# Ankur-Deka/Emergent-Multiagent-Strategies

Measured on AMD Instinct MI355X. Metric: env-steps/sec FortAttack 3v3, 4096 parallel envs per GPU, higher is better.
Workload: dtype f64

## Files before the change

emergent-multiagent-strategies_amd/build.py:

```python
import os
import shutil
import subprocess

CSRC = os.path.join(os.path.dirname(os.path.abspath(__file__)), "csrc")
ROOT = os.path.dirname(os.path.dirname(os.path.abspath(__file__)))
LIB = os.path.join(CSRC, "libfortattack_hip.so")
if os.environ.get("FA_LIBRARY"):
    LIB = os.path.abspath(os.environ["FA_LIBRARY"])
OBJ = os.path.join(CSRC, "_obj")
SOURCES = ["fa_step_pipe.hip", "fa_step_classic.hip", "fa_collect.hip", "fa_policy.hip", "fa_attend.hip", "fa_train.hip", "fa_train_dw.hip", "fa_fold.hip", "fa_rccl.hip", "fa_api.hip"]
FLAGS = ["--offload-arch=gfx950", "-O3", "-std=c++17", "-ffp-contract=off", "-fPIC", "-shared"]


def hipcc():
    return shutil.which("hipcc") or "/opt/rocm/bin/hipcc"


def needs_build():
    if os.environ.get("FA_LIBRARY"):
        return False
    if not os.path.isfile(LIB):
        return True
    deps = [os.path.join(CSRC, f) for f in SOURCES + ["fa_device.h", "fa_step_common.h", "experiments/fa_step_experiments.h", "fa_probe.h", "fa_policy.h", "fa_mfma.h", "fa_train.h"]]
    deps.append(os.path.join(ROOT, "include", "fortattack.h"))
    return any(os.path.getmtime(d) > os.path.getmtime(LIB) for d in deps)


def _load_mod(fname):
    import importlib.util
    spec = importlib.util.spec_from_file_location("_fa_" + fname[:-3], os.path.join(os.path.dirname(os.path.abspath(__file__)), fname))
    mod = importlib.util.module_from_spec(spec)
    spec.loader.exec_module(mod)
    return mod


def _load_lint():
    return _load_mod("isa_lint.py")


def _compile_one(src, verbose):
    isa_lint = _load_lint()
    base = os.path.join(OBJ, os.path.splitext(src)[0])
    common = [hipcc()] + [f for f in FLAGS if f != "-shared"] + ["-I", os.path.join(ROOT, "include")]
    cmd = common + ["-c", os.path.join(CSRC, src), "-o", base + ".o"]
    if verbose:
        print(" ".join(cmd))
    subprocess.check_call(cmd)
    subprocess.check_call(common + ["-S", "--cuda-device-only", os.path.join(CSRC, src), "-o", base + ".s"])
    bad = isa_lint.lint(base + ".s")
    if bad:
        raise RuntimeError("isa_lint: %s has %d vector instruction(s) ahead of an exec restore (a misplaced live-range "
                           "split: lanes that skipped the region lose the value), first: %s %s line %d: %s"
                           % (src, len(bad), bad[0][0], bad[0][1], bad[0][2][0], bad[0][2][1]))
    return base + ".o"


def build(force=False, verbose=False):
    if os.environ.get("FA_LIBRARY") or (not force and not needs_build()):
        return LIB
    from concurrent.futures import ThreadPoolExecutor
    os.makedirs(OBJ, exist_ok=True)
    with ThreadPoolExecutor(max_workers=4) as pool:
        objs = list(pool.map(lambda f: _compile_one(f, verbose), SOURCES))
    isa_model = _load_mod("isa_model.py")
    m = isa_model.write(os.path.join(OBJ, "fa_step_pipe.s"), os.path.join(OBJ, "fa_isa_model.json"))
    if os.environ.get("FA_ISA_REFRESH") == "1":
        isa_model.write(os.path.join(OBJ, "fa_step_pipe.s"))
    bad = isa_model.check(m)
    if bad:
        msg = "isa_model: the shipped step-kernel instantiations regressed: " + "; ".join(bad)
        if os.environ.get("FA_ISA_GATE", "1") == "0":
            import warnings
            warnings.warn(msg + "  (FA_ISA_GATE=0: building anyway)")
        else:
            if os.path.isfile(LIB):
                os.remove(LIB)
            raise RuntimeError(msg + "  (FA_ISA_GATE=0 builds anyway)")
    cmd = [hipcc(), "--offload-arch=gfx950", "-fPIC", "-shared"] + objs + ["-o", LIB]
    if verbose:
        print(" ".join(cmd))
    subprocess.check_call(cmd)
    return LIB


if __name__ == "__main__":
    print(build(force=True, verbose=True))
```

emergent-multiagent-strategies_amd/csrc/fa_mfma.h:

```cpp
#pragma once
#include <hip/hip_runtime.h>
#include <stdint.h>

#include "fa_policy.h"

#ifndef FA_GEMM_CH
#define FA_GEMM_CH 8
#endif
namespace {
constexpr int LDA = 132;
typedef float f32x16 __attribute__((ext_vector_type(16)));

template <int K>
struct BHead {
    static constexpr int NT = K / 8;
    static constexpr int CH = NT < FA_GEMM_CH ? NT : FA_GEMM_CH;
    float4 v[CH];
};
template <int K>
__device__ __forceinline__ void prefetch_b(const float4 *__restrict__ wp, int lane, BHead<K> &h) {
#pragma unroll
    for (int c = 0; c < BHead<K>::CH; ++c) h.v[c] = wp[c * 64 + lane];
}

template <int K, int NRB>
__device__ __forceinline__ void gemm_cb(const float *arow, const float4 *__restrict__ wp, f32x16 (&acc)[NRB], int lane,
                                        const BHead<K> &head) {
    constexpr int NT = BHead<K>::NT, CH = BHead<K>::CH;
    float4 bq[CH], bn[CH];
#pragma unroll
    for (int c = 0; c < CH; ++c) bq[c] = head.v[c];
#pragma unroll
    for (int t0 = 0; t0 < NT; t0 += CH) {
        if (t0 + CH < NT) {
#pragma unroll
            for (int c = 0; c < CH; ++c) bn[c] = wp[(t0 + CH + c) * 64 + lane];
#ifndef FA_NO_SCHED_BARRIER
            __builtin_amdgcn_sched_barrier(0);
#endif
        }
#pragma unroll
        for (int c = 0; c < CH; ++c) {
#pragma unroll
            for (int r = 0; r < NRB; ++r) {
                const float4 a = *reinterpret_cast<const float4 *>(arow + r * 32 * LDA + (t0 + c) * 4);
                acc[r] = __builtin_amdgcn_mfma_f32_32x32x2f32(a.x, bq[c].x, acc[r], 0, 0, 0);
                acc[r] = __builtin_amdgcn_mfma_f32_32x32x2f32(a.y, bq[c].y, acc[r], 0, 0, 0);
                acc[r] = __builtin_amdgcn_mfma_f32_32x32x2f32(a.z, bq[c].z, acc[r], 0, 0, 0);
                acc[r] = __builtin_amdgcn_mfma_f32_32x32x2f32(a.w, bq[c].w, acc[r], 0, 0, 0);
            }
        }
        if (t0 + CH < NT) {
#pragma unroll
            for (int c = 0; c < CH; ++c) bq[c] = bn[c];
        }
    }
}

#ifndef FA_GEMM3_CH
#define FA_GEMM3_CH 1
#endif
typedef __bf16 fa_bf16x8 __attribute__((ext_vector_type(8)));
typedef unsigned fa_u32x4 __attribute__((ext_vector_type(4)));
template <int K>
struct BHead3 {
    static constexpr int NS = K / 16;
    static constexpr int CH = NS < FA_GEMM3_CH ? NS : FA_GEMM3_CH;
    fa_u32x4 v[CH * 3];
};
template <int K>
__device__ __forceinline__ void prefetch_b3(const fa_u32x4 *__restrict__ wp, int lane, BHead3<K> &h) {
#pragma unroll
    for (int c = 0; c < BHead3<K>::CH * 3; ++c) h.v[c] = wp[c * 64 + lane];
}
__device__ __forceinline__ void fa_split8(const float4 &a0, const float4 &a1, fa_u32x4 &H, fa_u32x4 &M, fa_u32x4 &L) {
    const float x[8] = {a0.x, a0.y, a0.z, a0.w, a1.x, a1.y, a1.z, a1.w};
    unsigned h[8], m[8], l[8];
#pragma unroll
    for (int j = 0; j < 8; ++j) {
        h[j] = __float_as_uint(x[j]) & 0xffff0000u;
        const float r1 = x[j] - __uint_as_float(h[j]);
        m[j] = __float_as_uint(r1) & 0xffff0000u;
        l[j] = __float_as_uint(r1 - __uint_as_float(m[j]));
    }
#pragma unroll
    for (int j = 0; j < 4; ++j) {
        H[j] = __builtin_amdgcn_perm(h[2 * j + 1], h[2 * j], 0x07060302u);
        M[j] = __builtin_amdgcn_perm(m[2 * j + 1], m[2 * j], 0x07060302u);
        L[j] = __builtin_amdgcn_perm(l[2 * j + 1], l[2 * j], 0x07060302u);
    }
}
template <int K, int NRB>
__device__ __forceinline__ void gemm_cb3(const float *arow, const fa_u32x4 *__restrict__ wp3, f32x16 (&acc)[NRB], int lane,
                                         const BHead3<K> &head) {
    constexpr int NS = BHead3<K>::NS, CH = BHead3<K>::CH;
    fa_u32x4 bq[CH * 3], bn[CH * 3];
#pragma unroll
    for (int c = 0; c < CH * 3; ++c) bq[c] = head.v[c];
#pragma unroll
    for (int s0 = 0; s0 < NS; s0 += CH) {
        if (s0 + CH < NS) {
#pragma unroll
#ifdef FA_X3_KO_WLOAD
            for (int c = 0; c < CH * 3; ++c) bn[c] = bq[c] ^ (unsigned)s0;
#else
            for (int c = 0; c < CH * 3; ++c) bn[c] = wp3[((s0 + CH) * 3 + c) * 64 + lane];
#endif
#ifndef FA_NO_SCHED_BARRIER
            __builtin_amdgcn_sched_barrier(0);
#endif
        }
#pragma unroll
        for (int c = 0; c < CH; ++c) {
            const fa_bf16x8 bh = __builtin_bit_cast(fa_bf16x8, bq[c * 3]), bm = __builtin_bit_cast(fa_bf16x8, bq[c * 3 + 1]),
                            bl = __builtin_bit_cast(fa_bf16x8, bq[c * 3 + 2]);
#pragma unroll
            for (int r = 0; r < NRB; ++r) {
                const float *ap = arow + r * 32 * LDA + (s0 + c) * 8;
                fa_u32x4 H, M, L;
#ifdef FA_X3_KO_SPLIT
                H = __builtin_bit_cast(fa_u32x4, *reinterpret_cast<const float4 *>(ap));
                M = __builtin_bit_cast(fa_u32x4, *reinterpret_cast<const float4 *>(ap + 4));
                L = H ^ M;
#else
                fa_split8(*reinterpret_cast<const float4 *>(ap), *reinterpret_cast<const float4 *>(ap + 4), H, M, L);
#endif
                const fa_bf16x8 ah = __builtin_bit_cast(fa_bf16x8, H), am = __builtin_bit_cast(fa_bf16x8, M),
                                al = __builtin_bit_cast(fa_bf16x8, L);
                acc[r] = __builtin_amdgcn_mfma_f32_32x32x16_bf16(ah, bl, acc[r], 0, 0, 0);
                acc[r] = __builtin_amdgcn_mfma_f32_32x32x16_bf16(al, bh, acc[r], 0, 0, 0);
                acc[r] = __builtin_amdgcn_mfma_f32_32x32x16_bf16(am, bm, acc[r], 0, 0, 0);
                acc[r] = __builtin_amdgcn_mfma_f32_32x32x16_bf16(ah, bm, acc[r], 0, 0, 0);
                acc[r] = __builtin_amdgcn_mfma_f32_32x32x16_bf16(am, bh, acc[r], 0, 0, 0);
                acc[r] = __builtin_amdgcn_mfma_f32_32x32x16_bf16(ah, bh, acc[r], 0, 0, 0);
            }
#if !defined(FA_NO_SCHED_BARRIER) && !defined(FA_X3_NO_STEP_FENCE)
            __builtin_amdgcn_sched_barrier(0);
#endif
        }
        if (s0 + CH < NS) {
#pragma unroll
            for (int c = 0; c < CH * 3; ++c) bq[c] = bn[c];
        }
    }
}

template <bool RELU>
__device__ __forceinline__ void store_acc(float *dst, int rb, const f32x16 &acc, float bias, int lane) {
    const int col = lane & 31, hh = lane >> 5;
#pragma unroll
    for (int reg = 0; reg < 16; ++reg) {
        const int row = rb * 32 + (reg & 3) + 8 * (reg >> 2) + 4 * hh;
        float v = acc[reg] + bias;
        if (RELU) v = fmaxf(v, 0.0f);
        dst[row * LDA + col] = v;
    }
}

__device__ __forceinline__ float group16_sum(float v) {
#define FA_ROR_ADD(n) v += __builtin_bit_cast(float, __builtin_amdgcn_update_dpp(0, __builtin_bit_cast(int, v), 0x120 | (n), 0xf, 0xf, false))
    FA_ROR_ADD(8);
    FA_ROR_ADD(4);
    FA_ROR_ADD(2);
    FA_ROR_ADD(1);
#undef FA_ROR_ADD
    return v;
}

template <int W>
__device__ __forceinline__ void attend_row(const float *grow, const float *key0, int nk, int skip, float *orow, int q,
                                           float *attn_row = nullptr) {
    constexpr int C = W / 16;
    float gv[C];
#pragma unroll
    for (int c = 0; c < C; c += 4) *reinterpret_cast<float4 *>(gv + c) = *reinterpret_cast<const float4 *>(grow + q * C + c);
    float s[FA_POLICY_MAX_TEAM];
    float mx = -INFINITY;
#pragma unroll
    for (int j = 0; j < FA_POLICY_MAX_TEAM; ++j) {
        s[j] = -INFINITY;
        if (j < nk && j != skip) {
            float kv[C];
#pragma unroll
            for (int c = 0; c < C; c += 4)
                *reinterpret_cast<float4 *>(kv + c) = *reinterpret_cast<const float4 *>(key0 + j * LDA + q * C + c);
            float d = 0.0f;
#pragma unroll
            for (int c = 0; c < C; ++c) d = fmaf(gv[c], kv[c], d);
            s[j] = group16_sum(d);
            mx = fmaxf(mx, s[j]);
        }
    }
    float den = 0.0f;
#pragma unroll
    for (int j = 0; j < FA_POLICY_MAX_TEAM; ++j) {
        s[j] = (j < nk && j != skip) ? __expf(s[j] - mx) : 0.0f;
        den += s[j];
    }
    const float inv = den > 0.0f ? 1.0f / den : 0.0f;
    float ov[C];
#pragma unroll
    for (int c = 0; c < C; ++c) ov[c] = 0.0f;
#pragma unroll
    for (int j = 0; j < FA_POLICY_MAX_TEAM; ++j) {
        if (j < nk && j != skip) {
            const float a = s[j] * inv;
#pragma unroll
            for (int c = 0; c < C; c += 4) {
                const float4 kv = *reinterpret_cast<const float4 *>(key0 + j * LDA + q * C + c);
                ov[c] = fmaf(a, kv.x, ov[c]);
                ov[c + 1] = fmaf(a, kv.y, ov[c + 1]);
                ov[c + 2] = fmaf(a, kv.z, ov[c + 2]);
                ov[c + 3] = fmaf(a, kv.w, ov[c + 3]);
            }
        }
    }
#pragma unroll
    for (int c = 0; c < C; c += 4) *reinterpret_cast<float4 *>(orow + q * C + c) = *reinterpret_cast<const float4 *>(ov + c);
    if (attn_row && q < nk) {
        float aq = s[0];
#pragma unroll
        for (int j = 1; j < FA_POLICY_MAX_TEAM; ++j) aq = (j == q) ? s[j] : aq;
        attn_row[q] = aq * inv;
    }
}

template <int W, int MT>
__device__ __forceinline__ void attend_row_regs(const float *grow, const float *key0, int nk, int skip, int q, float (&ov)[W / 16],
                                                float *attn_row = nullptr) {
    constexpr int C = W / 16;
    float gv[C], kv[MT][C];
#pragma unroll
    for (int c = 0; c < C; c += 4) *reinterpret_cast<float4 *>(gv + c) = *reinterpret_cast<const float4 *>(grow + q * C + c);
#pragma unroll
    for (int j = 0; j < MT; ++j) {
#pragma unroll
        for (int c = 0; c < C; c += 4)
            *reinterpret_cast<float4 *>(&kv[j][c]) = j < nk ? *reinterpret_cast<const float4 *>(key0 + j * LDA + q * C + c) : float4{0, 0, 0, 0};
    }
    float s[MT], mx = -INFINITY;
#pragma unroll
    for (int j = 0; j < MT; ++j) {
        float d = 0.0f;
#pragma unroll
        for (int c = 0; c < C; ++c) d = fmaf(gv[c], kv[j][c], d);
        s[j] = group16_sum(d);
    }
#pragma unroll
    for (int j = 0; j < MT; ++j) {
        s[j] = (j < nk && j != skip) ? s[j] : -INFINITY;
        mx = fmaxf(mx, s[j]);
    }
    float den = 0.0f;
#pragma unroll
    for (int j = 0; j < MT; ++j) {
        s[j] = (j < nk && j != skip) ? __expf(s[j] - mx) : 0.0f;
        den += s[j];
    }
    const float inv = den > 0.0f ? 1.0f / den : 0.0f;
#pragma unroll
    for (int c = 0; c < C; ++c) ov[c] = 0.0f;
#pragma unroll
    for (int j = 0; j < MT; ++j) {
        if (j < nk) {
            const float a = s[j] * inv;
#pragma unroll
            for (int c = 0; c < C; ++c) ov[c] = fmaf(a, kv[j][c], ov[c]);
        }
    }
    if (attn_row && q < nk) {
        float aq = s[0];
#pragma unroll
        for (int j = 1; j < MT; ++j) aq = (j == q) ? s[j] : aq;
        attn_row[q] = aq * inv;
    }
}
template <int W>
__device__ __forceinline__ void store_row_regs(float *orow, int q, const float (&ov)[W / 16]) {
    constexpr int C = W / 16;
#pragma unroll
    for (int c = 0; c < C; c += 4) *reinterpret_cast<float4 *>(orow + q * C + c) = *reinterpret_cast<const float4 *>(ov + c);
}

}
```

emergent-multiagent-strategies_amd/csrc/fa_policy.hip:

```cpp
#include <hip/hip_runtime.h>
#include <stdint.h>
#include <type_traits>

#include "fa_policy.h"
#include "fa_mfma.h"
#define FA_PROBE_POLICY_TU
#include "fa_probe.h"

#ifndef FA_POLICY_WAVES
#define FA_POLICY_WAVES 8
#endif
#ifndef FA_POLICY_X3
#define FA_POLICY_X3 1
#endif
namespace {
#if FA_POLICY_X3
typedef fa_u32x4 pw_t;
template <int K> using PBHead = BHead3<K>;
template <int K> __device__ __forceinline__ void p_prefetch(const pw_t *__restrict__ wp, int lane, PBHead<K> &h) { prefetch_b3<K>(wp, lane, h); }
template <int K, int NRB>
__device__ __forceinline__ void p_gemm(const float *arow, const pw_t *__restrict__ wp, f32x16 (&acc)[NRB], int lane, const PBHead<K> &h) {
    gemm_cb3<K, NRB>(arow, wp, acc, lane, h);
}
#define FA_PW(OFF, OFF3, K, cb) (reinterpret_cast<const pw_t *>(W + (OFF3)) + (size_t)(cb) * ((K) / 16) * 3 * 64)
#else
typedef float4 pw_t;
template <int K> using PBHead = BHead<K>;
template <int K> __device__ __forceinline__ void p_prefetch(const pw_t *__restrict__ wp, int lane, PBHead<K> &h) { prefetch_b<K>(wp, lane, h); }
template <int K, int NRB>
__device__ __forceinline__ void p_gemm(const float *arow, const pw_t *__restrict__ wp, f32x16 (&acc)[NRB], int lane, const PBHead<K> &h) {
    gemm_cb<K, NRB>(arow, wp, acc, lane, h);
}
#define FA_PW(OFF, OFF3, K, cb) (reinterpret_cast<const pw_t *>(W + (OFF)) + (size_t)(cb) * ((K) / 8) * 64)
#endif
__device__ __forceinline__ void philox4x32_10(uint32_t c[4], uint32_t k0, uint32_t k1) {
#pragma unroll
    for (int r = 0; r < 10; ++r) {
        uint32_t hi0 = __umulhi(0xD2511F53u, c[0]), lo0 = 0xD2511F53u * c[0];
        uint32_t hi1 = __umulhi(0xCD9E8D57u, c[2]), lo1 = 0xCD9E8D57u * c[2];
        uint32_t n0 = hi1 ^ c[1] ^ k0, n2 = hi0 ^ c[3] ^ k1;
        c[0] = n0; c[1] = lo1; c[2] = n2; c[3] = lo0;
        k0 += 0x9E3779B9u; k1 += 0xBB67AE85u;
    }
}

#define FA_WAVES_BARRIER() asm volatile("s_waitcnt lgkmcnt(0)\n\ts_barrier" ::: "memory")
#define FA_POLICY_SPLIT(...)                                                          \
    if constexpr (NW == 8) {                                                          \
        if (wave < 4) { constexpr int R0 = 0, NR = 2; __VA_ARGS__ }                   \
        else { constexpr int R0 = 2, NR = 1; __VA_ARGS__ }                            \
    } else if constexpr (NW == 12) {                                                  \
        const int R0 = wave >> 2; constexpr int NR = 1; __VA_ARGS__                   \
    } else { constexpr int R0 = 0, NR = NRB; __VA_ARGS__ }
template <int NRB, int NW, bool ATTN>
__global__ __launch_bounds__(NW * 64, NRB == 2 ? 2 : 1) void fa_policy_kernel(FaPolicyArgs a) {
    static_assert((NRB == 3 && (NW == 8 || NW == 12)) || NW == 4, "eight / twelve waves: the 96-row tile");
    constexpr int PR = 32 * NRB;
    constexpr int NT = NW * 64;
    __shared__ __attribute__((aligned(16))) float sH[PR * LDA];
    __shared__ __attribute__((aligned(16))) float sG[PR * LDA];
    __shared__ float sX[PR * 2 * FA_OBS_DIM];
    __shared__ float sO[PR * 16];
    __shared__ float sNz[NW == 8 ? PR * FA_NUM_ACTIONS : 1];

    const int tid = threadIdx.x, lane = tid & 63, wave = __builtin_amdgcn_readfirstlane(tid >> 6);
    const int team = blockIdx.y;
    const int N = a.G + a.A;
    const int n = team == 0 ? a.G : a.A, m = N - n;
    const int own0 = team == 0 ? 0 : a.G, opp0 = team == 0 ? a.G : 0;
    const int ET = PR / (n > m ? n : m);
    const unsigned inv_n = 65536u / (unsigned)n + 1u, inv_m = 65536u / (unsigned)m + 1u;
    auto div_n = [&](int r) { return (int)(((unsigned)r * inv_n) >> 16); };
    auto div_m = [&](int r) { return (int)(((unsigned)r * inv_m) >> 16); };
    __shared__ int sE[PR];
    const float *W = a.w[team];
    if (a.env_list) {
        const int strat = a.tile_strategy[blockIdx.x];
        if (strat < 0) return;
        if (team == 1) W = a.pool + (size_t)strat * FA_POLICY_WEIGHT_FLOATS;
        if (tid < ET) sE[tid] = a.env_list[blockIdx.x * ET + tid];
    } else {
        const int e0 = blockIdx.x * ET;
        if (e0 >= a.E) return;
        if (tid < ET) sE[tid] = e0 + tid < a.E ? e0 + tid : -1;
    }
    float we[FA_OBS_DIM], wo[FA_OBS_DIM];
#pragma unroll
    for (int k = 0; k < FA_OBS_DIM; ++k) {
        we[k] = W[FA_POFF_WE + k * 64 + (tid & 63)];
        wo[k] = W[FA_POFF_WOE + k * 64 + (tid & 63)];
    }
    const float be = W[FA_POFF_BE + (tid & 63)], bo = W[FA_POFF_BOE + (tid & 63)];
    __syncthreads();

    for (int k = tid; k < ET * N * FA_OBS_DIM; k += NT) {
        const int el = k / (N * FA_OBS_DIM), e = sE[el];
        sX[k] = e >= 0 ? a.obs[(size_t)e * N * FA_OBS_DIM + (k - el * N * FA_OBS_DIM)] : 0.0f;
    }
    __syncthreads();

    FA_PL_TICK(0)
    const int li = lane & 31, hh = lane >> 5;
    const int cbw = wave & 3;
    const bool opp_two = NW == 4 && NRB == 3 && wave < 2;
    const bool opp_on = NW == 4 || wave < 2 * NRB;
    const int ocb = wave & 1, orb = NW >= 8 ? (wave >> 1) : (NRB == 3 ? 2 : (wave >> 1));
    const pw_t *wp_ao = FA_PW(FA_POFF_AO, FA_POFF3_AO, 64, ocb);
    const pw_t *wp_bo = FA_PW(FA_POFF_BO, FA_POFF3_BO, 64, ocb);
    const pw_t *wp_am = FA_PW(FA_POFF_AM, FA_POFF3_AM, 128, cbw);
    const pw_t *wp_w7 = FA_PW(FA_POFF_W7, FA_POFF3_W7, 256, cbw);
    const pw_t *wp_w8p = FA_PW(FA_POFF_W8, FA_POFF3_W8, 128, cbw);
    const pw_t *wp_w8v = FA_PW(FA_POFF_W8, FA_POFF3_W8, 128, 4 + cbw);
    const pw_t *wp_w9 = FA_PW(FA_POFF_W9, FA_POFF3_W9, 256, 0);
    PBHead<64> hd_o;
    if (opp_on) p_prefetch<64>(wp_ao, lane, hd_o);
    {
        const int col = tid & 63, grp = tid >> 6;
        for (int r = grp; r < PR; r += NW) {
            float vo = 0.0f, vp = 0.0f;
            if (r < ET * n) {
                const int el = div_n(r), i = r - el * n;
                const float *x = sX + (el * N + own0 + i) * FA_OBS_DIM;
                vo = be;
#pragma unroll
                for (int k = 0; k < FA_OBS_DIM; ++k) vo = fmaf(x[k], we[k], vo);
                vo = fmaxf(vo, 0.0f);
            }
            if (r < ET * m) {
                const int el = div_m(r), j = r - el * m;
                const float *x = sX + (el * N + opp0 + j) * FA_OBS_DIM;
                vp = bo;
#pragma unroll
                for (int k = 0; k < FA_OBS_DIM; ++k) vp = fmaf(x[k], wo[k], vp);
                vp = fmaxf(vp, 0.0f);
            }
            sH[r * LDA + col] = vo;
            sG[r * LDA + col] = vp;
        }
    }
    __syncthreads();
    FA_PL_TICK(1)

    if (opp_two) {
        f32x16 acc[2] = {};
        p_gemm<64, 2>(sH + li * LDA + hh * 32, wp_ao, acc, lane, hd_o);
        p_prefetch<64>(wp_bo, lane, hd_o);
        store_acc<false>(sG + 64 + ocb * 32, 0, acc[0], 0.0f, lane);
        store_acc<false>(sG + 64 + ocb * 32, 1, acc[1], 0.0f, lane);
    } else if (opp_on) {
        f32x16 acc[1] = {};
        p_gemm<64, 1>(sH + (orb * 32 + li) * LDA + hh * 32, wp_ao, acc, lane, hd_o);
        p_prefetch<64>(wp_bo, lane, hd_o);
        store_acc<false>(sG + 64 + ocb * 32, orb, acc[0], 0.0f, lane);
    }
    __syncthreads();
    FA_PL_TICK(2)
    constexpr int AIT = PR / (NW * 4);
    const int q16 = lane & 15, arow0 = wave * 4 + (lane >> 4), RU = ET * n;
    const bool small_teams = (n > m ? n : m) <= 4, mid_teams = (n > m ? n : m) <= 6;
    auto attn_dst = [&](float *base, int r, int nk) -> float * {
        if (!base || r >= RU) return nullptr;
        const int el = div_n(r), e = sE[el];
        return e >= 0 ? base + ((size_t)e * n + (r - el * n)) * nk : nullptr;
    };
    auto opp_attention = [&](auto MTc) __attribute__((always_inline)) {
        constexpr int MT = decltype(MTc)::value;
        float ov[AIT][4];
#pragma unroll
        for (int k = 0; k < AIT; ++k) {
            const int r = arow0 + k * NW * 4, rr = r < RU ? r : RU - 1;
            if constexpr (ATTN)
                attend_row_regs<64, MT>(sG + rr * LDA + 64, sG + (div_n(rr) * m) * LDA, m, -1, q16, ov[k], attn_dst(a.opp_attn[team], r, m));
            else
                attend_row_regs<64, MT>(sG + rr * LDA + 64, sG + (div_n(rr) * m) * LDA, m, -1, q16, ov[k]);
        }
#pragma unroll
        for (int k = 0; k < AIT; ++k) {
            const int r = arow0 + k * NW * 4;
            if (r < RU) store_row_regs<64>(sG + r * LDA + 64, q16, ov[k]);
        }
    };
    if (small_teams) opp_attention(std::integral_constant<int, 4>{});
    else if (mid_teams) opp_attention(std::integral_constant<int, 6>{});
    else opp_attention(std::integral_constant<int, FA_POLICY_MAX_TEAM>{});
    __syncthreads();
    FA_PL_TICK(3)
    PBHead<128> hd_m;
    if (opp_two) {
        f32x16 acc[2] = {};
        p_gemm<64, 2>(sG + li * LDA + 64 + hh * 32, wp_bo, acc, lane, hd_o);
        p_prefetch<128>(wp_am, lane, hd_m);
        store_acc<false>(sH + 64 + ocb * 32, 0, acc[0], 0.0f, lane);
        store_acc<false>(sH + 64 + ocb * 32, 1, acc[1], 0.0f, lane);
    } else if (opp_on) {
        f32x16 acc[1] = {};
        p_gemm<64, 1>(sG + (orb * 32 + li) * LDA + 64 + hh * 32, wp_bo, acc, lane, hd_o);
        p_prefetch<128>(wp_am, lane, hd_m);
        store_acc<false>(sH + 64 + ocb * 32, orb, acc[0], 0.0f, lane);
    } else {
        p_prefetch<128>(wp_am, lane, hd_m);
    }
    __syncthreads();

    auto team_attention = [&](auto MTc, [[maybe_unused]] float *attn_base) __attribute__((always_inline)) {
        constexpr int MT = decltype(MTc)::value;
        float ov[AIT][8];
#pragma unroll
        for (int k = 0; k < AIT; ++k) {
            const int r = arow0 + k * NW * 4, rr = r < RU ? r : RU - 1, el = div_n(rr);
            if constexpr (ATTN)
                attend_row_regs<128, MT>(sG + rr * LDA, sH + (el * n) * LDA, n, rr - el * n, q16, ov[k], attn_dst(attn_base, r, n));
            else
                attend_row_regs<128, MT>(sG + rr * LDA, sH + (el * n) * LDA, n, rr - el * n, q16, ov[k]);
        }
#pragma unroll
        for (int k = 0; k < AIT; ++k) {
            const int r = arow0 + k * NW * 4;
            if (r < RU) store_row_regs<128>(sG + r * LDA, q16, ov[k]);
        }
    };
    PBHead<256> hd_u;
    for (int round = 0; round < 3; ++round) {
        FA_PL_TICK(4 + round * 8)
        FA_POLICY_SPLIT({
            f32x16 acc[NR] = {};
            p_gemm<128, NR>(sH + (R0 * 32 + li) * LDA + hh * 64, wp_am, acc, lane, hd_m);
            p_prefetch<256>(wp_w7, lane, hd_u);
FA_PL_TICK(5 + round * 8)
_Pragma("unroll")
            for (int rb = 0; rb < NR; ++rb) store_acc<false>(sG + cbw * 32, R0 + rb, acc[rb], 0.0f, lane);
        })
        FA_PL_TICK(6 + round * 8)
        __syncthreads();
        FA_PL_TICK(7 + round * 8)
        float *const tattn = ATTN && round == 2 ? a.team_attn[team] : nullptr;
        if (small_teams) team_attention(std::integral_constant<int, 4>{}, tattn);
        else if (mid_teams) team_attention(std::integral_constant<int, 6>{}, tattn);
        else team_attention(std::integral_constant<int, FA_POLICY_MAX_TEAM>{}, tattn);
        FA_PL_TICK(8 + round * 8)
        __syncthreads();
        FA_PL_TICK(9 + round * 8)
        FA_POLICY_SPLIT({
            f32x16 acc[NR] = {};
            p_gemm<256, NR>((hh ? sG : sH) + (R0 * 32 + li) * LDA, wp_w7, acc, lane, hd_u);
            p_prefetch<128>(round < 2 ? wp_am : wp_w8p, lane, hd_m);
            const float bias = W[FA_POFF_BU + cbw * 32 + li];
            FA_PL_TICK(10 + round * 8)
            FA_WAVES_BARRIER();
            FA_PL_TICK(11 + round * 8)
_Pragma("unroll")
            for (int rb = 0; rb < NR; ++rb) store_acc<true>(sH + cbw * 32, R0 + rb, acc[rb], bias, lane);
        })
        __syncthreads();
    }

    FA_PL_TICK(28)
    FA_POLICY_SPLIT({
        PBHead<128> hd_v;
        p_prefetch<128>(wp_w8v, lane, hd_v);
        {
            f32x16 accp[NR] = {};
            p_gemm<128, NR>(sH + (R0 * 32 + li) * LDA + hh * 64, wp_w8p, accp, lane, hd_m);
            const float bp = W[FA_POFF_B8 + cbw * 32 + li];
_Pragma("unroll")
            for (int rb = 0; rb < NR; ++rb) store_acc<true>(sG + cbw * 32, R0 + rb, accp[rb], bp, lane);
        }
        f32x16 accv[NR] = {};
        p_gemm<128, NR>(sH + (R0 * 32 + li) * LDA + hh * 64, wp_w8v, accv, lane, hd_v);
        if (wave < NRB) p_prefetch<256>(wp_w9, lane, hd_u);
        const float bv = W[FA_POFF_B8 + 128 + cbw * 32 + li];
        FA_WAVES_BARRIER();
_Pragma("unroll")
        for (int rb = 0; rb < NR; ++rb) store_acc<true>(sH + cbw * 32, R0 + rb, accv[rb], bv, lane);
    })
    __syncthreads();
    FA_PL_TICK(29)
    auto gumbel_row = [&](int row, float (&g)[FA_NUM_ACTIONS]) __attribute__((always_inline)) {
        const int el = div_n(row), i = row - el * n;
        const uint64_t ge = (uint64_t)(a.env_offset + sE[el]);
        const uint32_t ctr = a.counter ? (uint32_t)a.counter[0] : 0u;
#pragma unroll
        for (int half = 0; half < 2; ++half) {
            uint32_t c[4] = {(uint32_t)ge, (uint32_t)(ge >> 32) ^ ((uint32_t)(own0 + i) << 16) ^ ((uint32_t)half << 31),
                             (uint32_t)a.step, ctr};
            philox4x32_10(c, (uint32_t)a.seed, (uint32_t)(a.seed >> 32));
#pragma unroll
            for (int k = 0; k < 4; ++k) {
                const float u = ((float)(c[k] >> 8) + 0.5f) * (1.0f / 16777216.0f);
                g[half * 4 + k] = logf(-logf(u));
            }
        }
    };
    if (NW == 8 && wave >= 4 && wave < 6 && !a.deterministic && !a.value_only) {
        const int row = tid - 256;
        if (row < RU && sE[div_n(row)] >= 0) {
            float g[FA_NUM_ACTIONS];
            gumbel_row(row, g);
#pragma unroll
            for (int k = 0; k < FA_NUM_ACTIONS; ++k) sNz[row * FA_NUM_ACTIONS + k] = g[k];
        }
    }
    if (wave < NRB) {
        f32x16 acc[1] = {};
        p_gemm<256, 1>((hh ? sH : sG) + (wave * 32 + li) * LDA, wp_w9, acc, lane, hd_u);
        if (li < 16) {
            const float bias = W[FA_POFF_B9 + li];
#pragma unroll
            for (int reg = 0; reg < 16; ++reg) {
                const int row = wave * 32 + (reg & 3) + 8 * (reg >> 2) + 4 * hh;
                sO[row * 16 + li] = acc[0][reg] + bias;
            }
        }
    }
    __syncthreads();
    FA_PL_TICK(30)

    const int el_out = tid < PR ? div_n(tid) : 0;
    if (tid < ET * n && sE[el_out] >= 0) {
        const int el = el_out, i = tid - el * n;
        const int e = sE[el];
        const size_t o = (size_t)e * N + own0 + i;
        const float *lo = sO + tid * 16;
        if (a.value) a.value[o] = lo[8];
        if (!a.value_only) {
            float lg[FA_NUM_ACTIONS], mx = -INFINITY;
#pragma unroll
            for (int k = 0; k < FA_NUM_ACTIONS; ++k) { lg[k] = lo[k]; mx = fmaxf(mx, lg[k]); }
            float se = 0.0f;
#pragma unroll
            for (int k = 0; k < FA_NUM_ACTIONS; ++k) se += expf(lg[k] - mx);
            const float lse = mx + logf(se);
            int act = 0;
            if (a.deterministic) {
                float best = lg[0];
#pragma unroll
                for (int k = 1; k < FA_NUM_ACTIONS; ++k)
                    if (lg[k] > best) { best = lg[k]; act = k; }
            } else {
                float g[FA_NUM_ACTIONS];
                if constexpr (NW == 8) {
#pragma unroll
                    for (int k = 0; k < FA_NUM_ACTIONS; ++k) g[k] = sNz[tid * FA_NUM_ACTIONS + k];
                } else {
                    gumbel_row(tid, g);
                }
                float best = -INFINITY;
#pragma unroll
                for (int k = 0; k < FA_NUM_ACTIONS; ++k) {
                    const float z = lg[k] - g[k];
                    if (z > best) { best = z; act = k; }
                }
            }
            float la = lg[0];
#pragma unroll
            for (int k = 1; k < FA_NUM_ACTIONS; ++k) la = (k == act) ? lg[k] : la;
            a.action[o] = (int64_t)act;
            a.logp[o] = la - lse;
        }
    }
    FA_PL_TICK(31)
}
#undef FA_POLICY_SPLIT
__global__ __launch_bounds__(1024) void fa_group_envs_kernel(const int32_t *__restrict__ strat, int E, int K, int ET, int tiles_max,
                                                            int32_t *__restrict__ env_list, int32_t *__restrict__ tile_strategy) {
    __shared__ int cnt[FA_POLICY_MAX_POOL], start[FA_POLICY_MAX_POOL], cur[FA_POLICY_MAX_POOL];
    const int tid = threadIdx.x;
    if (tid < FA_POLICY_MAX_POOL) { cnt[tid] = 0; cur[tid] = 0; }
    __syncthreads();
    auto clampk = [&](int k) { return k < 0 ? 0 : (k >= K ? K - 1 : k); };
    for (int e = tid; e < E; e += blockDim.x) atomicAdd(&cnt[clampk(strat[e])], 1);
    for (int s = tid; s < tiles_max * ET; s += blockDim.x) env_list[s] = -1;
    __syncthreads();
    if (tid == 0) {
        int t = 0;
        for (int k = 0; k < K; ++k) {
            start[k] = t * ET;
            const int nt = (cnt[k] + ET - 1) / ET;
            for (int j = 0; j < nt && t + j < tiles_max; ++j) tile_strategy[t + j] = k;
            t += nt;
        }
        for (; t < tiles_max; ++t) tile_strategy[t] = -1;
    }
    __syncthreads();
    for (int e = tid; e < E; e += blockDim.x) {
        const int k = clampk(strat[e]);
        env_list[start[k] + atomicAdd(&cur[k], 1)] = e;
    }
}
}

static int policy_rows(int E, int G, int A) {
    const int n_max = G > A ? G : A, et96 = FA_POLICY_ROWS / n_max;
    const int wgs96 = 2 * ((E + et96 - 1) / et96);
    return wgs96 < 192 ? 64 : FA_POLICY_ROWS;
}
int fa_policy_tile_envs(int E, int G, int A) { return policy_rows(E, G, A) / (G > A ? G : A); }

hipError_t fa_launch_group_envs(const int32_t *env_strategy, int E, int pool_size, int G, int A, int32_t *env_list,
                                int32_t *tile_strategy, int tiles_max, hipStream_t st) {
    hipLaunchKernelGGL(fa_group_envs_kernel, dim3(1), dim3(1024), 0, st, env_strategy, E, pool_size, fa_policy_tile_envs(E, G, A),
                       tiles_max, env_list, tile_strategy);
    return hipGetLastError();
}

hipError_t fa_launch_policy(const FaPolicyArgs &a, hipStream_t st) {
    const int ET = fa_policy_tile_envs(a.E, a.G, a.A);
    const int tiles = a.env_list ? a.tiles : (a.E + ET - 1) / ET;
    const bool attn = a.team_attn[0] || a.team_attn[1] || a.opp_attn[0] || a.opp_attn[1];
    const bool rows64 = policy_rows(a.E, a.G, a.A) == 64;
    if (rows64 && !attn) hipLaunchKernelGGL((fa_policy_kernel<2, 4, false>), dim3(tiles, 2), dim3(256), 0, st, a);
    else if (rows64) hipLaunchKernelGGL((fa_policy_kernel<2, 4, true>), dim3(tiles, 2), dim3(256), 0, st, a);
    else if (!attn) hipLaunchKernelGGL((fa_policy_kernel<3, FA_POLICY_WAVES, false>), dim3(tiles, 2), dim3(FA_POLICY_WAVES * 64), 0, st, a);
    else hipLaunchKernelGGL((fa_policy_kernel<3, FA_POLICY_WAVES, true>), dim3(tiles, 2), dim3(FA_POLICY_WAVES * 64), 0, st, a);
    return hipGetLastError();
}
```

Measured before the change: 3.140 billion.

## Store policy activations in LDS as pre-split bf16x3 planes for MFMA

Policy-kernel activation buffers in LDS switch from a padded fp32 row layout to three bf16 planes (hi/mid/lo) in 16-byte chunks. The hi/mid/lo split now happens once when each activation is stored, instead of inside every GEMM A-operand load. Stores pair rows via a DPP lane swap, and attention reads rebuild fp32 values from the planes. This adds split work on every store and a join on every attention read, and changes the LDS footprint and access pattern, which could affect bank conflicts and occupancy.

Measured after the change: 3.140 billion (median of 2 runs). No clear change (-0.0%).

```diff
diff --git a/emergent-multiagent-strategies_amd/build.py b/emergent-multiagent-strategies_amd/build.py
--- a/emergent-multiagent-strategies_amd/build.py
+++ b/emergent-multiagent-strategies_amd/build.py
@@ -21,7 +21,7 @@
         return False
     if not os.path.isfile(LIB):
         return True
-    deps = [os.path.join(CSRC, f) for f in SOURCES + ["fa_device.h", "fa_step_common.h", "experiments/fa_step_experiments.h", "fa_probe.h", "fa_policy.h", "fa_mfma.h", "fa_train.h"]]
+    deps = [os.path.join(CSRC, f) for f in SOURCES + ["fa_device.h", "fa_step_common.h", "experiments/fa_step_experiments.h", "fa_probe.h", "fa_policy.h", "fa_mfma.h", "fa_planes.h", "fa_train.h"]]
     deps.append(os.path.join(ROOT, "include", "fortattack.h"))
     return any(os.path.getmtime(d) > os.path.getmtime(LIB) for d in deps)
 
diff --git a/emergent-multiagent-strategies_amd/csrc/fa_mfma.h b/emergent-multiagent-strategies_amd/csrc/fa_mfma.h
--- a/emergent-multiagent-strategies_amd/csrc/fa_mfma.h
+++ b/emergent-multiagent-strategies_amd/csrc/fa_mfma.h
@@ -3,6 +3,7 @@
 #include <stdint.h>
 
 #include "fa_policy.h"
+#include "fa_planes.h"
 
 #ifndef FA_GEMM_CH
 #define FA_GEMM_CH 8
@@ -282,4 +283,179 @@
     for (int c = 0; c < C; c += 4) *reinterpret_cast<float4 *>(orow + q * C + c) = *reinterpret_cast<const float4 *>(ov + c);
 }
 
-}
+typedef unsigned fa_u32x2 __attribute__((ext_vector_type(2)));
+
+template <int K, int NRB>
+__device__ __forceinline__ void gemm_cb3p(const fa_u32x4 *ap, const fa_u32x4 *__restrict__ wp3, f32x16 (&acc)[NRB], int lane,
+                                          const BHead3<K> &head) {
+    constexpr int NS = BHead3<K>::NS, CH = BHead3<K>::CH;
+    fa_u32x4 bq[CH * 3], bn[CH * 3];
+#pragma unroll
+    for (int c = 0; c < CH * 3; ++c) bq[c] = head.v[c];
+#pragma unroll
+    for (int s0 = 0; s0 < NS; s0 += CH) {
+        if (s0 + CH < NS) {
+#pragma unroll
+#ifdef FA_X3_KO_WLOAD
+            for (int c = 0; c < CH * 3; ++c) bn[c] = bq[c] ^ (unsigned)s0;
+#else
+            for (int c = 0; c < CH * 3; ++c) bn[c] = wp3[((s0 + CH) * 3 + c) * 64 + lane];
+#endif
+#ifndef FA_NO_SCHED_BARRIER
+            __builtin_amdgcn_sched_barrier(0);
+#endif
+        }
+#pragma unroll
+        for (int c = 0; c < CH; ++c) {
+            const fa_bf16x8 bh = __builtin_bit_cast(fa_bf16x8, bq[c * 3]), bm = __builtin_bit_cast(fa_bf16x8, bq[c * 3 + 1]),
+                            bl = __builtin_bit_cast(fa_bf16x8, bq[c * 3 + 2]);
+#pragma unroll
+            for (int r = 0; r < NRB; ++r) {
+                const fa_u32x4 *p = ap + (s0 + c) * FA_PLANE_S + r * 32;
+                const fa_bf16x8 ah = __builtin_bit_cast(fa_bf16x8, p[0]), am = __builtin_bit_cast(fa_bf16x8, p[FA_PLANE_CHUNKS]),
+                                al = __builtin_bit_cast(fa_bf16x8, p[2 * FA_PLANE_CHUNKS]);
+                acc[r] = __builtin_amdgcn_mfma_f32_32x32x16_bf16(ah, bl, acc[r], 0, 0, 0);
+                acc[r] = __builtin_amdgcn_mfma_f32_32x32x16_bf16(al, bh, acc[r], 0, 0, 0);
+                acc[r] = __builtin_amdgcn_mfma_f32_32x32x16_bf16(am, bm, acc[r], 0, 0, 0);
+                acc[r] = __builtin_amdgcn_mfma_f32_32x32x16_bf16(ah, bm, acc[r], 0, 0, 0);
+                acc[r] = __builtin_amdgcn_mfma_f32_32x32x16_bf16(am, bh, acc[r], 0, 0, 0);
+                acc[r] = __builtin_amdgcn_mfma_f32_32x32x16_bf16(ah, bh, acc[r], 0, 0, 0);
+            }
+#if !defined(FA_NO_SCHED_BARRIER) && defined(FA_X3P_STEP_FENCE)
+            __builtin_amdgcn_sched_barrier(0);
+#endif
+        }
+        if (s0 + CH < NS) {
+#pragma unroll
+            for (int c = 0; c < CH * 3; ++c) bq[c] = bn[c];
+        }
+    }
+}
+
+__device__ __forceinline__ void plane_store_pair(fa_u32x4 *buf, int rowA, int rowB, int col, float vA, float vB) {
+    const bool odd = col & 1;
+    const float send = odd ? vA : vB;
+    const float recv = __builtin_bit_cast(float, __builtin_amdgcn_update_dpp(0, __builtin_bit_cast(int, send), 0xB1 ,
+                                                                             0xf, 0xf, false));
+    const float c0 = odd ? recv : vA, c1 = odd ? vB : recv;
+    uint32_t h0, m0, l0, h1, m1, l1;
+    fa_split3(c0, h0, m0, l0);
+    fa_split3(c1, h1, m1, l1);
+    unsigned *d = reinterpret_cast<unsigned *>(buf + fa_plane_chunk(0, col >> 3, odd ? rowB : rowA)) + ((col & 7) >> 1);
+    d[0] = fa_pack_hi16(h0, h1);
+    d[FA_PLANE_CHUNKS * 4] = fa_pack_hi16(m0, m1);
+    d[2 * FA_PLANE_CHUNKS * 4] = fa_pack_hi16(l0, l1);
+}
+template <bool RELU>
+__device__ __forceinline__ void store_acc_p(fa_u32x4 *buf, int col0, int rb, const f32x16 &acc, float bias, int lane) {
+    const int col = col0 + (lane & 31), hh = lane >> 5;
+#pragma unroll
+    for (int i = 0; i < 8; ++i) {
+        const int row = rb * 32 + (i & 3) + 8 * (i >> 2) + 4 * hh;
+        float vA = acc[i] + bias, vB = acc[i + 8] + bias;
+        if (RELU) { vA = fmaxf(vA, 0.0f); vB = fmaxf(vB, 0.0f); }
+        plane_store_pair(buf, row, row + 16, col, vA, vB);
+    }
+}
+
+template <int C>
+__device__ __forceinline__ void plane_load_row(const fa_u32x4 *buf, int row, int col0, float (&x)[C]) {
+    static_assert(C == 8 || C == 4, "a chunk or half a chunk");
+    unsigned H[C / 2], M[C / 2], L[C / 2];
+    if constexpr (C == 8) {
+        const fa_u32x4 *p = buf + fa_plane_chunk(0, col0 >> 3, row);
+        const fa_u32x4 h = p[0], m = p[FA_PLANE_CHUNKS], l = p[2 * FA_PLANE_CHUNKS];
+#pragma unroll
+        for (int j = 0; j < 4; ++j) { H[j] = h[j]; M[j] = m[j]; L[j] = l[j]; }
+    } else {
+        const fa_u32x2 *p = reinterpret_cast<const fa_u32x2 *>(buf + fa_plane_chunk(0, col0 >> 3, row)) + ((col0 >> 2) & 1);
+        const fa_u32x2 h = p[0], m = p[FA_PLANE_CHUNKS * 2], l = p[2 * FA_PLANE_CHUNKS * 2];
+#pragma unroll
+        for (int j = 0; j < 2; ++j) { H[j] = h[j]; M[j] = m[j]; L[j] = l[j]; }
+    }
+#pragma unroll
+    for (int j = 0; j < C / 2; ++j) {
+        x[2 * j] = fa_join3(fa_plane_lo_col(H[j]), fa_plane_lo_col(M[j]), fa_plane_lo_col(L[j]));
+        x[2 * j + 1] = fa_join3(fa_plane_hi_col(H[j]), fa_plane_hi_col(M[j]), fa_plane_hi_col(L[j]));
+    }
+}
+template <int C>
+__device__ __forceinline__ void plane_store_row(fa_u32x4 *buf, int row, int col0, const float (&x)[C]) {
+    static_assert(C == 8 || C == 4, "a chunk or half a chunk");
+    unsigned H[C / 2], M[C / 2], L[C / 2];
+#pragma unroll
+    for (int j = 0; j < C / 2; ++j) {
+        uint32_t h0, m0, l0, h1, m1, l1;
+        fa_split3(x[2 * j], h0, m0, l0);
+        fa_split3(x[2 * j + 1], h1, m1, l1);
+        H[j] = fa_pack_hi16(h0, h1);
+        M[j] = fa_pack_hi16(m0, m1);
+        L[j] = fa_pack_hi16(l0, l1);
+    }
+    if constexpr (C == 8) {
+        fa_u32x4 *p = buf + fa_plane_chunk(0, col0 >> 3, row);
+        p[0] = fa_u32x4{H[0], H[1], H[2], H[3]};
+        p[FA_PLANE_CHUNKS] = fa_u32x4{M[0], M[1], M[2], M[3]};
+        p[2 * FA_PLANE_CHUNKS] = fa_u32x4{L[0], L[1], L[2], L[3]};
+    } else {
+        fa_u32x2 *p = reinterpret_cast<fa_u32x2 *>(buf + fa_plane_chunk(0, col0 >> 3, row)) + ((col0 >> 2) & 1);
+        p[0] = fa_u32x2{H[0], H[1]};
+        p[FA_PLANE_CHUNKS * 2] = fa_u32x2{M[0], M[1]};
+        p[2 * FA_PLANE_CHUNKS * 2] = fa_u32x2{L[0], L[1]};
+    }
+}
+
+template <int W, int MT>
+__device__ __forceinline__ void attend_row_regs_p(const fa_u32x4 *gbuf, int grow, int gcol, const fa_u32x4 *kbuf, int krow0, int kcol,
+                                                  int nk, int skip, int q, float (&ov)[W / 16], float *attn_row = nullptr) {
+    constexpr int C = W / 16;
+    float gv[C], kv[MT][C];
+    plane_load_row<C>(gbuf, grow, gcol + q * C, gv);
+#pragma unroll
+    for (int j = 0; j < MT; ++j) {
+        if (j < nk) {
+            plane_load_row<C>(kbuf, krow0 + j, kcol + q * C, kv[j]);
+        } else {
+#pragma unroll
+            for (int c = 0; c < C; ++c) kv[j][c] = 0.0f;
+        }
+    }
+    float s[MT], mx = -INFINITY;
+#pragma unroll
+    for (int j = 0; j < MT; ++j) {
+        float d = 0.0f;
+#pragma unroll
+        for (int c = 0; c < C; ++c) d = fmaf(gv[c], kv[j][c], d);
+        s[j] = group16_sum(d);
+    }
+#pragma unroll
+    for (int j = 0; j < MT; ++j) {
+        s[j] = (j < nk && j != skip) ? s[j] : -INFINITY;
+        mx = fmaxf(mx, s[j]);
+    }
+    float den = 0.0f;
+#pragma unroll
+    for (int j = 0; j < MT; ++j) {
+        s[j] = (j < nk && j != skip) ? __expf(s[j] - mx) : 0.0f;
+        den += s[j];
+    }
+    const float inv = den > 0.0f ? 1.0f / den : 0.0f;
+#pragma unroll
+    for (int c = 0; c < C; ++c) ov[c] = 0.0f;
+#pragma unroll
+    for (int j = 0; j < MT; ++j) {
+        if (j < nk) {
+            const float a = s[j] * inv;
+#pragma unroll
+            for (int c = 0; c < C; ++c) ov[c] = fmaf(a, kv[j][c], ov[c]);
+        }
+    }
+    if (attn_row && q < nk) {
+        float aq = s[0];
+#pragma unroll
+        for (int j = 1; j < MT; ++j) aq = (j == q) ? s[j] : aq;
+        attn_row[q] = aq * inv;
+    }
+}
+
+}
diff --git a/emergent-multiagent-strategies_amd/csrc/fa_planes.h b/emergent-multiagent-strategies_amd/csrc/fa_planes.h
--- /dev/null
+++ b/emergent-multiagent-strategies_amd/csrc/fa_planes.h
@@ -0,0 +1,43 @@
+#pragma once
+#include <stdint.h>
+
+#if defined(__HIPCC__) || defined(__CUDACC__)
+#define FA_PLANES_FN __host__ __device__ inline
+#else
+#define FA_PLANES_FN inline
+#endif
+
+constexpr int FA_PLANE_ROWS = 96;
+constexpr int FA_PLANE_COLS = 128;
+constexpr int FA_PLANE_S = 97;
+constexpr int FA_PLANE_CC = FA_PLANE_COLS / 8;
+constexpr int FA_PLANE_CHUNKS = FA_PLANE_CC * FA_PLANE_S;
+constexpr int FA_PLANE_BUF_CHUNKS = 3 * FA_PLANE_CHUNKS;
+constexpr int FA_PLANE_BUF_BYTES = FA_PLANE_BUF_CHUNKS * 16;
+constexpr int FA_PLANE_LDS_LIMIT = 160 * 1024;
+constexpr FA_PLANES_FN int fa_plane_tile_lds_bytes(int obs_dim, int num_actions) {
+    return 2 * FA_PLANE_BUF_BYTES + FA_PLANE_ROWS * 4 * (2 * obs_dim + 16 + num_actions + 1);
+}
+
+constexpr FA_PLANES_FN int fa_plane_chunk(int p, int c, int row) { return p * FA_PLANE_CHUNKS + c * FA_PLANE_S + row; }
+constexpr FA_PLANES_FN int fa_plane_byte(int p, int row, int col) { return fa_plane_chunk(p, col >> 3, row) * 16 + (col & 7) * 2; }
+
+FA_PLANES_FN uint32_t fa_f2u(float x) { return __builtin_bit_cast(uint32_t, x); }
+FA_PLANES_FN float fa_u2f(uint32_t u) { return __builtin_bit_cast(float, u); }
+
+FA_PLANES_FN void fa_split3(float x, uint32_t &h, uint32_t &m, uint32_t &l) {
+    h = fa_f2u(x) & 0xffff0000u;
+    const float r1 = x - fa_u2f(h);
+    m = fa_f2u(r1) & 0xffff0000u;
+    l = fa_f2u(r1 - fa_u2f(m));
+}
+FA_PLANES_FN uint32_t fa_pack_hi16(uint32_t lo_col, uint32_t hi_col) {
+#if defined(__HIP_DEVICE_COMPILE__)
+    return __builtin_amdgcn_perm(hi_col, lo_col, 0x07060302u);
+#else
+    return (lo_col >> 16) | (hi_col & 0xffff0000u);
+#endif
+}
+FA_PLANES_FN float fa_plane_lo_col(uint32_t d) { return fa_u2f(d << 16); }
+FA_PLANES_FN float fa_plane_hi_col(uint32_t d) { return fa_u2f(d & 0xffff0000u); }
+FA_PLANES_FN float fa_join3(float h, float m, float l) { return (h + m) + l; }
diff --git a/emergent-multiagent-strategies_amd/csrc/fa_policy.hip b/emergent-multiagent-strategies_amd/csrc/fa_policy.hip
--- a/emergent-multiagent-strategies_amd/csrc/fa_policy.hip
+++ b/emergent-multiagent-strategies_amd/csrc/fa_policy.hip
@@ -33,6 +33,46 @@
 }
 #define FA_PW(OFF, OFF3, K, cb) (reinterpret_cast<const pw_t *>(W + (OFF)) + (size_t)(cb) * ((K) / 8) * 64)
 #endif
+#ifndef FA_POLICY_PLANES
+#define FA_POLICY_PLANES 1
+#endif
+template <int NRB, int NW>
+constexpr bool kPlanes = FA_POLICY_PLANES && FA_POLICY_X3 && NRB == 3 && NW == 8;
+
+__device__ __forceinline__ const float *a_ptr(const float *buf, int row, int col) { return buf + row * LDA + col; }
+__device__ __forceinline__ const fa_u32x4 *a_ptr(const fa_u32x4 *buf, int row, int col) { return buf + fa_plane_chunk(0, col >> 3, row); }
+#if FA_POLICY_X3
+template <int K, int NRB>
+__device__ __forceinline__ void p_gemm(const fa_u32x4 *ap, const pw_t *__restrict__ wp, f32x16 (&acc)[NRB], int lane, const PBHead<K> &h) {
+    gemm_cb3p<K, NRB>(ap, wp, acc, lane, h);
+}
+#endif
+template <bool RELU>
+__device__ __forceinline__ void p_store_acc(float *buf, int col0, int rb, const f32x16 &acc, float bias, int lane) {
+    store_acc<RELU>(buf + col0, rb, acc, bias, lane);
+}
+template <bool RELU>
+__device__ __forceinline__ void p_store_acc(fa_u32x4 *buf, int col0, int rb, const f32x16 &acc, float bias, int lane) {
+    store_acc_p<RELU>(buf, col0, rb, acc, bias, lane);
+}
+template <int W, int MT>
+__device__ __forceinline__ void p_attend(const float *gbuf, int grow, int gcol, const float *kbuf, int krow0, int kcol, int nk, int skip,
+                                         int q, float (&ov)[W / 16], float *attn_row) {
+    attend_row_regs<W, MT>(gbuf + grow * LDA + gcol, kbuf + krow0 * LDA + kcol, nk, skip, q, ov, attn_row);
+}
+template <int W, int MT>
+__device__ __forceinline__ void p_attend(const fa_u32x4 *gbuf, int grow, int gcol, const fa_u32x4 *kbuf, int krow0, int kcol, int nk,
+                                         int skip, int q, float (&ov)[W / 16], float *attn_row) {
+    attend_row_regs_p<W, MT>(gbuf, grow, gcol, kbuf, krow0, kcol, nk, skip, q, ov, attn_row);
+}
+template <int W>
+__device__ __forceinline__ void p_store_row(float *buf, int row, int col0, int q, const float (&ov)[W / 16]) {
+    store_row_regs<W>(buf + row * LDA + col0, q, ov);
+}
+template <int W>
+__device__ __forceinline__ void p_store_row(fa_u32x4 *buf, int row, int col0, int q, const float (&ov)[W / 16]) {
+    plane_store_row<W / 16>(buf, row, col0 + q * (W / 16), ov);
+}
 __device__ __forceinline__ void philox4x32_10(uint32_t c[4], uint32_t k0, uint32_t k1) {
 #pragma unroll
     for (int r = 0; r < 10; ++r) {
@@ -57,11 +97,18 @@
     static_assert((NRB == 3 && (NW == 8 || NW == 12)) || NW == 4, "eight / twelve waves: the 96-row tile");
     constexpr int PR = 32 * NRB;
     constexpr int NT = NW * 64;
-    __shared__ __attribute__((aligned(16))) float sH[PR * LDA];
-    __shared__ __attribute__((aligned(16))) float sG[PR * LDA];
+    constexpr bool PL = kPlanes<NRB, NW>;
+    static_assert(!PL || (PR == FA_PLANE_ROWS && FA_POLICY_X3), "planes: the 96-row tile of the bf16x3 form only");
+    using abuf_t = std::conditional_t<PL, fa_u32x4, float>;
+    constexpr int ABUF = PL ? FA_PLANE_BUF_CHUNKS : PR * LDA;
+    __shared__ __attribute__((aligned(16))) abuf_t sH[ABUF];
+    __shared__ __attribute__((aligned(16))) abuf_t sG[ABUF];
     __shared__ float sX[PR * 2 * FA_OBS_DIM];
     __shared__ float sO[PR * 16];
     __shared__ float sNz[NW == 8 ? PR * FA_NUM_ACTIONS : 1];
+    constexpr int LDS_BYTES = 2 * sizeof(abuf_t) * ABUF + sizeof(float) * (PR * 2 * FA_OBS_DIM + PR * 16 + PR * FA_NUM_ACTIONS) + sizeof(int) * PR;
+    static_assert(!PL || (LDS_BYTES == fa_plane_tile_lds_bytes(FA_OBS_DIM, FA_NUM_ACTIONS) && LDS_BYTES <= FA_PLANE_LDS_LIMIT),
+                  "the 96-row tile's LDS");
 
     const int tid = threadIdx.x, lane = tid & 63, wave = __builtin_amdgcn_readfirstlane(tid >> 6);
     const int team = blockIdx.y;
@@ -116,8 +163,8 @@
     if (opp_on) p_prefetch<64>(wp_ao, lane, hd_o);
     {
         const int col = tid & 63, grp = tid >> 6;
-        for (int r = grp; r < PR; r += NW) {
-            float vo = 0.0f, vp = 0.0f;
+        auto enc_row = [&](int r, float &vo, float &vp) __attribute__((always_inline)) {
+            vo = 0.0f, vp = 0.0f;
             if (r < ET * n) {
                 const int el = div_n(r), i = r - el * n;
                 const float *x = sX + (el * N + own0 + i) * FA_OBS_DIM;
@@ -134,8 +181,23 @@
                 for (int k = 0; k < FA_OBS_DIM; ++k) vp = fmaf(x[k], wo[k], vp);
                 vp = fmaxf(vp, 0.0f);
             }
-            sH[r * LDA + col] = vo;
-            sG[r * LDA + col] = vp;
+        };
+        if constexpr (PL) {
+            static_assert(PR % (2 * NW) == 0, "row pairs (r, r + NW)");
+            for (int r = grp; r < PR; r += 2 * NW) {
+                float vo0, vp0, vo1, vp1;
+                enc_row(r, vo0, vp0);
+                enc_row(r + NW, vo1, vp1);
+                plane_store_pair(sH, r, r + NW, col, vo0, vo1);
+                plane_store_pair(sG, r, r + NW, col, vp0, vp1);
+            }
+        } else {
+            for (int r = grp; r < PR; r += NW) {
+                float vo, vp;
+                enc_row(r, vo, vp);
+                sH[r * LDA + col] = vo;
+                sG[r * LDA + col] = vp;
+            }
         }
     }
     __syncthreads();
@@ -143,15 +205,15 @@
 
     if (opp_two) {
         f32x16 acc[2] = {};
-        p_gemm<64, 2>(sH + li * LDA + hh * 32, wp_ao, acc, lane, hd_o);
+        p_gemm<64, 2>(a_ptr(sH, li, hh * 32), wp_ao, acc, lane, hd_o);
         p_prefetch<64>(wp_bo, lane, hd_o);
-        store_acc<false>(sG + 64 + ocb * 32, 0, acc[0], 0.0f, lane);
-        store_acc<false>(sG + 64 + ocb * 32, 1, acc[1], 0.0f, lane);
+        p_store_acc<false>(sG, 64 + ocb * 32, 0, acc[0], 0.0f, lane);
+        p_store_acc<false>(sG, 64 + ocb * 32, 1, acc[1], 0.0f, lane);
     } else if (opp_on) {
         f32x16 acc[1] = {};
-        p_gemm<64, 1>(sH + (orb * 32 + li) * LDA + hh * 32, wp_ao, acc, lane, hd_o);
+        p_gemm<64, 1>(a_ptr(sH, orb * 32 + li, hh * 32), wp_ao, acc, lane, hd_o);
         p_prefetch<64>(wp_bo, lane, hd_o);
-        store_acc<false>(sG + 64 + ocb * 32, orb, acc[0], 0.0f, lane);
+        p_store_acc<false>(sG, 64 + ocb * 32, orb, acc[0], 0.0f, lane);
     }
     __syncthreads();
     FA_PL_TICK(2)
@@ -170,14 +232,14 @@
         for (int k = 0; k < AIT; ++k) {
             const int r = arow0 + k * NW * 4, rr = r < RU ? r : RU - 1;
             if constexpr (ATTN)
-                attend_row_regs<64, MT>(sG + rr * LDA + 64, sG + (div_n(rr) * m) * LDA, m, -1, q16, ov[k], attn_dst(a.opp_attn[team], r, m));
+                p_attend<64, MT>(sG, rr, 64, sG, div_n(rr) * m, 0, m, -1, q16, ov[k], attn_dst(a.opp_attn[team], r, m));
             else
-                attend_row_regs<64, MT>(sG + rr * LDA + 64, sG + (div_n(rr) * m) * LDA, m, -1, q16, ov[k]);
+                p_attend<64, MT>(sG, rr, 64, sG, div_n(rr) * m, 0, m, -1, q16, ov[k], nullptr);
         }
 #pragma unroll
         for (int k = 0; k < AIT; ++k) {
             const int r = arow0 + k * NW * 4;
-            if (r < RU) store_row_regs<64>(sG + r * LDA + 64, q16, ov[k]);
+            if (r < RU) p_store_row<64>(sG, r, 64, q16, ov[k]);
         }
     };
     if (small_teams) opp_attention(std::integral_constant<int, 4>{});
@@ -188,15 +250,15 @@
     PBHead<128> hd_m;
     if (opp_two) {
         f32x16 acc[2] = {};
-        p_gemm<64, 2>(sG + li * LDA + 64 + hh * 32, wp_bo, acc, lane, hd_o);
+        p_gemm<64, 2>(a_ptr(sG, li, 64 + hh * 32), wp_bo, acc, lane, hd_o);
         p_prefetch<128>(wp_am, lane, hd_m);
-        store_acc<false>(sH + 64 + ocb * 32, 0, acc[0], 0.0f, lane);
-        store_acc<false>(sH + 64 + ocb * 32, 1, acc[1], 0.0f, lane);
+        p_store_acc<false>(sH, 64 + ocb * 32, 0, acc[0], 0.0f, lane);
+        p_store_acc<false>(sH, 64 + ocb * 32, 1, acc[1], 0.0f, lane);
     } else if (opp_on) {
         f32x16 acc[1] = {};
-        p_gemm<64, 1>(sG + (orb * 32 + li) * LDA + 64 + hh * 32, wp_bo, acc, lane, hd_o);
+        p_gemm<64, 1>(a_ptr(sG, orb * 32 + li, 64 + hh * 32), wp_bo, acc, lane, hd_o);
         p_prefetch<128>(wp_am, lane, hd_m);
-        store_acc<false>(sH + 64 + ocb * 32, orb, acc[0], 0.0f, lane);
+        p_store_acc<false>(sH, 64 + ocb * 32, orb, acc[0], 0.0f, lane);
     } else {
         p_prefetch<128>(wp_am, lane, hd_m);
     }
@@ -209,14 +271,14 @@
         for (int k = 0; k < AIT; ++k) {
             const int r = arow0 + k * NW * 4, rr = r < RU ? r : RU - 1, el = div_n(rr);
             if constexpr (ATTN)
-                attend_row_regs<128, MT>(sG + rr * LDA, sH + (el * n) * LDA, n, rr - el * n, q16, ov[k], attn_dst(attn_base, r, n));
+                p_attend<128, MT>(sG, rr, 0, sH, el * n, 0, n, rr - el * n, q16, ov[k], attn_dst(attn_base, r, n));
             else
-                attend_row_regs<128, MT>(sG + rr * LDA, sH + (el * n) * LDA, n, rr - el * n, q16, ov[k]);
+                p_attend<128, MT>(sG, rr, 0, sH, el * n, 0, n, rr - el * n, q16, ov[k], nullptr);
         }
 #pragma unroll
         for (int k = 0; k < AIT; ++k) {
             const int r = arow0 + k * NW * 4;
-            if (r < RU) store_row_regs<128>(sG + r * LDA, q16, ov[k]);
+            if (r < RU) p_store_row<128>(sG, r, 0, q16, ov[k]);
         }
     };
     PBHead<256> hd_u;
@@ -224,11 +286,11 @@
         FA_PL_TICK(4 + round * 8)
         FA_POLICY_SPLIT({
             f32x16 acc[NR] = {};
-            p_gemm<128, NR>(sH + (R0 * 32 + li) * LDA + hh * 64, wp_am, acc, lane, hd_m);
+            p_gemm<128, NR>(a_ptr(sH, R0 * 32 + li, hh * 64), wp_am, acc, lane, hd_m);
             p_prefetch<256>(wp_w7, lane, hd_u);
 FA_PL_TICK(5 + round * 8)
 _Pragma("unroll")
-            for (int rb = 0; rb < NR; ++rb) store_acc<false>(sG + cbw * 32, R0 + rb, acc[rb], 0.0f, lane);
+            for (int rb = 0; rb < NR; ++rb) p_store_acc<false>(sG, cbw * 32, R0 + rb, acc[rb], 0.0f, lane);
         })
         FA_PL_TICK(6 + round * 8)
         __syncthreads();
@@ -242,14 +304,14 @@
         FA_PL_TICK(9 + round * 8)
         FA_POLICY_SPLIT({
             f32x16 acc[NR] = {};
-            p_gemm<256, NR>((hh ? sG : sH) + (R0 * 32 + li) * LDA, wp_w7, acc, lane, hd_u);
+            p_gemm<256, NR>(a_ptr(hh ? sG : sH, R0 * 32 + li, 0), wp_w7, acc, lane, hd_u);
             p_prefetch<128>(round < 2 ? wp_am : wp_w8p, lane, hd_m);
             const float bias = W[FA_POFF_BU + cbw * 32 + li];
             FA_PL_TICK(10 + round * 8)
             FA_WAVES_BARRIER();
             FA_PL_TICK(11 + round * 8)
 _Pragma("unroll")
-            for (int rb = 0; rb < NR; ++rb) store_acc<true>(sH + cbw * 32, R0 + rb, acc[rb], bias, lane);
+            for (int rb = 0; rb < NR; ++rb) p_store_acc<true>(sH, cbw * 32, R0 + rb, acc[rb], bias, lane);
         })
         __syncthreads();
     }
@@ -260,18 +322,18 @@
         p_prefetch<128>(wp_w8v, lane, hd_v);
         {
             f32x16 accp[NR] = {};
-            p_gemm<128, NR>(sH + (R0 * 32 + li) * LDA + hh * 64, wp_w8p, accp, lane, hd_m);
+            p_gemm<128, NR>(a_ptr(sH, R0 * 32 + li, hh * 64), wp_w8p, accp, lane, hd_m);
             const float bp = W[FA_POFF_B8 + cbw * 32 + li];
 _Pragma("unroll")
-            for (int rb = 0; rb < NR; ++rb) store_acc<true>(sG + cbw * 32, R0 + rb, accp[rb], bp, lane);
+            for (int rb = 0; rb < NR; ++rb) p_store_acc<true>(sG, cbw * 32, R0 + rb, accp[rb], bp, lane);
         }
         f32x16 accv[NR] = {};
-        p_gemm<128, NR>(sH + (R0 * 32 + li) * LDA + hh * 64, wp_w8v, accv, lane, hd_v);
+        p_gemm<128, NR>(a_ptr(sH, R0 * 32 + li, hh * 64), wp_w8v, accv, lane, hd_v);
         if (wave < NRB) p_prefetch<256>(wp_w9, lane, hd_u);
         const float bv = W[FA_POFF_B8 + 128 + cbw * 32 + li];
         FA_WAVES_BARRIER();
 _Pragma("unroll")
-        for (int rb = 0; rb < NR; ++rb) store_acc<true>(sH + cbw * 32, R0 + rb, accv[rb], bv, lane);
+        for (int rb = 0; rb < NR; ++rb) p_store_acc<true>(sH, cbw * 32, R0 + rb, accv[rb], bv, lane);
     })
     __syncthreads();
     FA_PL_TICK(29)
@@ -302,7 +364,7 @@
     }
     if (wave < NRB) {
         f32x16 acc[1] = {};
-        p_gemm<256, 1>((hh ? sH : sG) + (wave * 32 + li) * LDA, wp_w9, acc, lane, hd_u);
+        p_gemm<256, 1>(a_ptr(hh ? sH : sG, wave * 32 + li, 0), wp_w9, acc, lane, hd_u);
         if (li < 16) {
             const float bias = W[FA_POFF_B9 + li];
 #pragma unroll
```
